# Kaz-K/medical-image-editing

Measured on AMD Instinct MI355X. Metric: images/sec (train step, 256x256 2D slices), higher is better.
Workload: dtype f32

## Files before the change

medical-image-editing_amd/csrc/conv_wino64.hip:

```cpp
#include "common.h"
#include "conv_common.h"
#include "mfma_util.h"
#include "wino_common.h"

extern int g_wino_mode;

namespace {

struct W64Args {
    const float* x;
    const float* u;
    const float* bias;
    float* y;
    int N, H, W, Cin, Cout;
    int tilesY, tilesX, nsp;
    int ntn, nch;
    int kt;
    int relu;
    unsigned nbx, nbu, nby;
    float* stats;
    const float* mask;
    const float* mr;
    int in_relu;
    float* y2;
    int split, pool0;
    int c1;
    unsigned nby2;
    unsigned img_px, rowb_px, rpx, ppx;
    int n_sh, n_m;
};

constexpr int W6_KPH = wino::KPH;
template <int RW, int MBW, int NW = 8> struct W64Geo {
    static_assert(MBW == 1 || (MBW == 2 && RW == 32), "two M blocks per wave: 32-wide regions only");
    static_assert(NW == 8 || (NW == 4 && RW == 32), "four-wave workgroups: 32-wide regions only");
    static constexpr int NMB = NW / 2;
    static constexpr int NBW = 4 / MBW;
    static constexpr int NCO = 16 * NBW;
    static constexpr int TR = RW == 32 ? 2 * MBW * NMB : 16;
    static constexpr int HR = TR + 2, HWV = RW + 2;
    static constexpr int HWS = RW == 32 ? 34 : 24;
    static constexpr int HBUF = HR * HWS * W6_KPH;
    static constexpr int UBUF = 16 * NCO * 8;
    static constexpr int EXF = 2048 * NW;
    static_assert(EXF >= UBUF, "U buffer 1 lives in the exchange area");
    static constexpr size_t LDS_FLOATS = 2 * HBUF + UBUF + EXF + 2 * NMB * NCO * 2;
};
constexpr int W6_LS = 4;
constexpr int W6_ULS = 2;
constexpr int W6_CP = 48;

template <int RW, int MBW, int EPI, int NW = 8>
__global__ void __launch_bounds__(64 * NW, 8 / NW) k_conv_wino64(W64Args a) {
    constexpr bool MASK = EPI >= 1 && EPI <= 3;
    using G = W64Geo<RW, MBW, NW>;
    constexpr int NT = 64 * NW, NMB = G::NMB, NBW = G::NBW, NCO = G::NCO;
    constexpr int HWS = G::HWS, HWV = G::HWV, HBUF = G::HBUF, UBUF = G::UBUF;
    using Halo = wino::HaloStager<NT, G::HR, HWV, HWS, wino::PitchedPix>;
    constexpr int LH = Halo::LH;
    constexpr int LU = 512 * NBW / NT;
    constexpr int HP0 = 1 + LU * W6_ULS;
    static_assert(HP0 + (LH - 1) * W6_LS < W6_CP && W6_CP + LH <= 64, "prefetch slots fit the item");

    extern __shared__ __attribute__((aligned(16))) float smem[];
    float* Hs = smem;
    float* Us = smem + 2 * HBUF;
    float* Ex = Us + UBUF;
    float* Rs = Ex + G::EXF;

    const int tid = threadIdx.x, lane = tid & 63;
    const int wv = __builtin_amdgcn_readfirstlane(tid >> 6);
    const int mb = wv & (NMB - 1), h = wv / NMB;
    const int H = a.H, W = a.W, Cin = a.Cin, Cout = a.Cout;
    const __amdgpu_buffer_rsrc_t rsx = make_rsrc(a.x, a.nbx), rsu = make_rsrc(a.u, a.nbu), rsy = make_rsrc(a.y, a.nby);
    const __amdgpu_buffer_rsrc_t rsm = make_rsrc((EPI == 1 || EPI == 3) ? a.mask : a.y, a.nby);
    const __amdgpu_buffer_rsrc_t rsr = make_rsrc(EPI == 3 ? a.mr : a.y, EPI == 3 ? (unsigned)((size_t)a.N * a.Cout * 8) : a.nby);
    const __amdgpu_buffer_rsrc_t rsy2 = make_rsrc(EPI == 4 ? a.y2 : a.y, EPI == 4 ? a.nby2 : a.nby);

    const int nch = a.nch;
    const wino::RegionRun run = wino::region_run(a.ntn, a.kt, a.nsp);
    const int co_base = run.tile_n * NCO;
    const int my_tiles = run.my_tiles;
    if (my_tiles <= 0) return;

    const int c4 = tid & 1;
    const wino::PitchedPix pixel = {a.img_px, a.rowb_px, a.rpx, a.ppx, a.n_sh, a.n_m};
    Halo hs;
    hs.init(tid, pixel);
    auto region_offsets = [&](int n, int tx, int ty) { hs.region_offsets(n, ty * G::TR - 1, tx * RW - 1, H, W, Cin); };
    const int u_n = (tid >> 1) & (NCO - 1);
    const int u_swz = (u_n >> 3) & 1;
    const int u_c4 = c4 ^ u_swz;
    const unsigned u_voff = (((unsigned)(tid >> 1) / NCO * Cout + co_base + u_n) * 8u + u_c4 * 4) * 4u;
    const unsigned u_jstride = (unsigned)(NT / 2 / NCO) * Cout * 32u;
    const unsigned u_cstride = 16u * Cout * 32u;
    const int u_wave = wv * 256;

    auto issue_h = [&](int j, int chunk) { hs.issue_h(rsx, j, chunk); };
    auto commit_h = [&](int j, float* Hb) { hs.commit_h(j, Hb); };
    auto issue_u = [&](int j, int chunk, float* Ub) {
        wino::buf_ld4_lds(rsu, Ub + u_wave + j * (NT * 4), u_voff, chunk * u_cstride + j * u_jstride);
    };

    int cn, ctx, cty, ch = 0;
    region_start(run.sp0, a.tilesY, a.tilesX, cn, ctx, cty);
    auto advance = [&](int& n, int& tx, int& ty, int& c) {
        const int adv = c + 1 == nch ? 1 : 0;
        c = adv ? 0 : c + 1;
        region_step(adv, a.tilesY, a.tilesX, n, tx, ty);
    };
    int n1 = cn, tx1 = ctx, ty1 = cty, ch1 = 0;
    advance(n1, tx1, ty1, ch1);
    int n2 = n1, tx2 = tx1, ty2 = ty1, ch2 = ch1;
    advance(n2, tx2, ty2, ch2);
    auto shift = [&]() {
        cn = n1; ctx = tx1; cty = ty1; ch = ch1;
        n1 = n2; tx1 = tx2; ty1 = ty2; ch1 = ch2;
        advance(n2, tx2, ty2, ch2);
    };

    const int m = lane & 15, q = lane >> 4;
    const int rA = h ? 3 : 0, rB = h ? 2 : 1, rC = h ? 1 : 2;
    const int prow = RW == 32 ? 2 * MBW * mb : 2 * (2 * mb + (m >> 3)), pcol = RW == 32 ? 2 * m : 2 * (m & 7);
    constexpr int MBW_STEP = 2 * HWS * W6_KPH;
    const int a_A = opaque(((prow + rA) * HWS + pcol) * W6_KPH + 2 * q);
    const int a_B = opaque(((prow + rB) * HWS + pcol) * W6_KPH + 2 * q);
    const int a_C = opaque(((prow + rC) * HWS + pcol) * W6_KPH + 2 * q);
    const int b_swz = ((q >> 1) ^ (m >> 3)) * 4 + (q & 1) * 2;
    const int b_0 = opaque(((h ? 3 : 0) * 4 * NCO + m) * 8 + b_swz);
    const int b_1 = opaque(((h ? 2 : 1) * 4 * NCO + m) * 8 + b_swz);
    const float sg = opaque_f(h ? -1.f : 1.f), mone = opaque_f(-1.f);

    f32x4 acc[8][MBW][NBW];
    f32x2 bf[2][NBW];
    f32x2 dcol[2][3];
    float e[2][2][4];
    float v[2][MBW][2][8];

    auto read_col = [&](const float* Hb, int w, int c) {
        const float* Hc = Hb + w * MBW_STEP + c * W6_KPH;
        dcol[c & 1][0] = *(const f32x2*)&Hc[a_A];
        dcol[c & 1][1] = *(const f32x2*)&Hc[a_B];
        dcol[c & 1][2] = *(const f32x2*)&Hc[a_C];
    };
    auto xform_op = [&](int par, int w, int o) {
        if (o < 16) {
            const int c = o >> 2, k = o & 3, t = k >> 1;
            const float dA = dcol[c & 1][0][t], dB = dcol[c & 1][1][t], dC = dcol[c & 1][2][t];
            if ((k & 1) == 0) e[t][0][c] = __builtin_fmaf(mone, dC, dA);
            else e[t][1][c] = __builtin_fmaf(sg, dC, dB);
        } else {
            const int k = o - 16, lr = k >> 3, t = (k >> 2) & 1, cc = k & 3;
            const float e0 = e[t][lr][0], e1 = e[t][lr][1], e2 = e[t][lr][2], e3 = e[t][lr][3];
            v[par][w][t][lr * 4 + cc] = wino::bt_row_plain(cc, e0, e1, e2, e3);
        }
    };
    auto xform_slot = [&](const float* Hn, int par, int p) {
        constexpr int NOPS = 32 * MBW, P0 = MBW == 1 ? 32 : 4;
        auto op = [&](int g) { xform_op(par, g >> 5, g & 31); };
        auto rd = [&](int g) {
            if ((g & 31) < 16 && ((g & 31) & 3) == 0) read_col(Hn, g >> 5, (g & 31) >> 2);
        };
        if (p + 3 - P0 >= 0 && p + 3 - P0 < NOPS) rd(p + 3 - P0);
        if (p - P0 >= 0 && p - P0 < NOPS && p < 64) {
            const int g = p - P0;
            if (P0 + NOPS <= 64 || g < NOPS - 2 * (P0 + NOPS - 64)) op(g);
            else { const int d = g - (NOPS - 2 * (P0 + NOPS - 64)); op(NOPS - 2 * (P0 + NOPS - 64) + 2 * d); op(NOPS - 2 * (P0 + NOPS - 64) + 2 * d + 1); }
        }
    };

    region_offsets(cn, ctx, cty);
#pragma unroll
    for (int j = 0; j < LH; ++j) issue_h(j, 0);
#pragma unroll
    for (int j = 0; j < LU; ++j) issue_u(j, 0, Us);
#pragma unroll
    for (int j = 0; j < LH; ++j) commit_h(j, Hs);
    region_offsets(n1, tx1, ty1);
#pragma unroll
    for (int j = 0; j < LH; ++j) issue_h(j, ch1);
#pragma unroll
    for (int j = 0; j < LH; ++j) commit_h(j, Hs + HBUF);
    wino::dma_wait();
    __syncthreads();
#pragma unroll
    for (int w = 0; w < MBW; ++w)
#pragma unroll
        for (int o = 0; o < 32; ++o) {
            if (o < 16 && (o & 3) == 0) read_col(Hs, w, o >> 2);
            xform_op(0, w, o);
        }
    __syncthreads();
    region_offsets(n2, tx2, ty2);

    float bvv[NBW / 2];
#pragma unroll
    for (int i = 0; i < NBW / 2; ++i) bvv[i] = a.bias ? a.bias[co_base + (h * (NBW / 2) + i) * 16 + m] : 0.f;
    const float lo = a.relu ? 0.f : -__builtin_inff();
    const bool plain = a.bias == nullptr && !a.relu;
    int spar = 0;

    auto body = [&](auto PAR, auto FIRST) {
        constexpr int par = decltype(PAR)::value;
        constexpr bool first = decltype(FIRST)::value;
        const float* Uc = Us + par * UBUF;
        const float* Hn = Hs + (par ^ 1) * HBUF;
        float* Hw = Hs + par * HBUF;
        float* Uw = Us + (par ^ 1) * UBUF;
        auto ldb = [&](int l, int nb) {
            bf[l & 1][nb] = *(const f32x2*)&Uc[(l < 4 ? b_0 : b_1) + ((l & 3) * NCO + nb * 16) * 8];
        };
        static_assert(par == 0 || (par ^ 1) == 0, "a region's last item (odd) loads U into buffer 0: buffer 1 is the epilogue's exchange area");
        auto slot = [&](int p) {
            if (p >= 1 && p < HP0 && (p - 1) % W6_ULS == 0) issue_u((p - 1) / W6_ULS, ch1, Uw);
            if (p >= HP0 && p < HP0 + LH * W6_LS && (p - HP0) % W6_LS == 0) issue_h((p - HP0) / W6_LS, ch2);
            if (p >= W6_CP && p < W6_CP + LH) commit_h(p - W6_CP, Hw);
            xform_slot(Hn, par ^ 1, p);
        };
#pragma unroll
        for (int nb = 0; nb < NBW; ++nb) { ldb(0, nb); __builtin_amdgcn_sched_barrier(0); }
        const f32x4 zero4 = {0.f, 0.f, 0.f, 0.f};
        if (first) {
#pragma unroll
            for (int p = 0; p < 8; ++p) slot(p);
#pragma unroll
            for (int w = 0; w < MBW; ++w)
#pragma unroll
                for (int nb = 0; nb < NBW; ++nb) acc[7][w][nb] = zero4;
        } else {
#pragma unroll
            for (int j = 0; j < 8; ++j) {
                const int w = j / (2 * NBW), k = (j / NBW) & 1, nb = j % NBW;
                acc[7][w][nb] = MFMA16(v[par ^ 1][w][k][7], k == 0 ? bf[1][nb].x : bf[1][nb].y, acc[7][w][nb]);
                slot(j);
                __builtin_amdgcn_sched_barrier(0);
            }
        }
#pragma unroll
        for (int l = 0; l < 7; ++l) {
#pragma unroll
            for (int j = 0; j < 8; ++j) {
                const int w = j / (2 * NBW), k = (j / NBW) & 1, nb = j % NBW;
                if (j < NBW) ldb(l + 1, nb);
                acc[l][w][nb] = MFMA16(v[par][w][k][l], k == 0 ? bf[l & 1][nb].x : bf[l & 1][nb].y, (first && k == 0) ? zero4 : acc[l][w][nb]);
                slot(8 + l * 8 + j);
                __builtin_amdgcn_sched_barrier(0);
            }
        }
    };
    auto flush = [&]() {
#pragma unroll
        for (int j = 0; j < 8; ++j) {
            const int w = j / (2 * NBW), k = (j / NBW) & 1, nb = j % NBW;
            acc[7][w][nb] = MFMA16(v[1][w][k][7], k == 0 ? bf[1][nb].x : bf[1][nb].y, acc[7][w][nb]);
            __builtin_amdgcn_sched_barrier(0);
        }
    };

    auto partial = [&](auto HH, int w, int nb, int r, float* yv) {
        constexpr int hh = decltype(HH)::value;
        float p0[4], p1[4];
#pragma unroll
        for (int j = 0; j < 4; ++j) {
            const float l0 = acc[j][w][nb][r], l1 = acc[4 + j][w][nb][r];
            if (hh == 0) { p0[j] = l0 + l1; p1[j] = l1; }
            else { p0[j] = l1; p1[j] = l0 - l1; }
        }
        yv[0] = (p0[0] + p0[1]) + p0[2];
        yv[1] = (p0[1] - p0[2]) - p0[3];
        yv[2] = (p1[0] + p1[1]) + p1[2];
        yv[3] = (p1[1] - p1[2]) - p1[3];
    };
    auto epi_send = [&](auto HH) {
        constexpr int hh = decltype(HH)::value;
        float* Xo = Ex + (((mb * 2 + (hh ^ 1)) * 8) * 64 + lane) * 4;
#pragma unroll
        for (int w = 0; w < MBW; ++w)
#pragma unroll
            for (int i = 0; i < NBW / 2; ++i)
#pragma unroll
                for (int r = 0; r < 4; ++r) {
                    float yv[4];
                    partial(HH, w, (hh ^ 1) * (NBW / 2) + i, r, yv);
                    float4 o;
                    o.x = yv[0]; o.y = yv[1]; o.z = yv[2]; o.w = yv[3];
                    *(float4*)&Xo[((w * (NBW / 2) + i) * 4 + r) * 256] = o;
                }
    };
    auto epi_finish = [&](auto HH) {
        constexpr int hh = decltype(HH)::value;
        const float* Xi = Ex + (((mb * 2 + hh) * 8) * 64 + lane) * 4;
        float st1[NBW / 2], st2[NBW / 2];
#pragma unroll
        for (int w = 0; w < MBW; ++w) {
            const int yrow0 = cty * G::TR + (RW == 32 ? 2 * (MBW * mb + w) : 2 * (2 * mb + (q >> 1)));
            const int xcol0 = ctx * RW + (RW == 32 ? 8 * q : 8 * (q & 1));
#pragma unroll
            for (int i = 0; i < NBW / 2; ++i) {
                float yv[16];
                const int co0 = co_base + (hh * (NBW / 2) + i) * 16;
                const unsigned co = (unsigned)(co0 + m);
                const bool part0 = EPI == 4 && co0 < a.split;
                const bool pooled = part0 && a.pool0;
                const unsigned cs = EPI != 4 ? (unsigned)Cout : (unsigned)(part0 ? a.split : a.c1);
                const unsigned cc = EPI != 4 ? co : (part0 ? co : co - (unsigned)a.split);
                int voffs[2];
#pragma unroll
                for (int aa = 0; aa < 2; ++aa) {
                    const int yy = yrow0 + aa;
                    const unsigned base = (pixel.base(cn) + (unsigned)yy * a.rpx + (unsigned)xcol0 * a.ppx) * cs + cc;
                    voffs[aa] = (int)sel_u32(yy < H, base * 4u, 0xFFFFFFFFu);
                }
                float mk[16];
                if (MASK) {
#pragma unroll
                    for (int aa = 0; aa < 2; ++aa)
#pragma unroll
                        for (int r = 0; r < 4; ++r)
#pragma unroll
                            for (int b = 0; b < 2; ++b)
                                mk[r * 4 + aa * 2 + b] = __uint_as_float(__builtin_amdgcn_raw_buffer_load_b32(rsm, voffs[aa], (2 * r + b) * (int)a.ppx * Cout * 4, 0));
                }
#pragma unroll
                for (int r = 0; r < 4; ++r) {
                    float own[4];
                    partial(HH, w, hh * (NBW / 2) + i, r, own);
                    const float4 o = *(const float4*)&Xi[((w * (NBW / 2) + i) * 4 + r) * 256];
                    if (plain) {
                        yv[r * 4 + 0] = own[0] + o.x; yv[r * 4 + 1] = own[1] + o.y;
                        yv[r * 4 + 2] = own[2] + o.z; yv[r * 4 + 3] = own[3] + o.w;
                    } else {
                        yv[r * 4 + 0] = fmaxf((own[0] + o.x) + bvv[i], lo);
                        yv[r * 4 + 1] = fmaxf((own[1] + o.y) + bvv[i], lo);
                        yv[r * 4 + 2] = fmaxf((own[2] + o.z) + bvv[i], lo);
                        yv[r * 4 + 3] = fmaxf((own[3] + o.w) + bvv[i], lo);
                    }
                }
                if (EPI == 1) {
#pragma unroll
                    for (int k = 0; k < 16; ++k) yv[k] = mk[k] > 0.f ? yv[k] : 0.f;
                } else if (EPI == 2) {
#pragma unroll
                    for (int k = 0; k < 16; ++k) yv[k] = mk[k] + yv[k];
                } else if (EPI == 3) {
                    const unsigned mo = ((unsigned)(cn >> a.n_sh) * (unsigned)Cout + co) * 8u;
                    const float mean = __uint_as_float(__builtin_amdgcn_raw_buffer_load_b32(rsr, (int)mo, 0, 0));
                    const float rstd = __uint_as_float(__builtin_amdgcn_raw_buffer_load_b32(rsr, (int)mo, 4, 0));
                    float s1 = 0.f, s2 = 0.f;
#pragma unroll
                    for (int k = 0; k < 16; ++k) {
                        const float xh = (mk[k] - mean) * rstd;
                        const float gm = (a.in_relu && !(xh > 0.f)) ? 0.f : yv[k];
                        s1 += gm;
                        s2 = __builtin_fmaf(gm, xh, s2);
                    }
                    s1 += __shfl_xor(s1, 16, 64); s2 += __shfl_xor(s2, 16, 64);
                    s1 += __shfl_xor(s1, 32, 64); s2 += __shfl_xor(s2, 32, 64);
                    if (w == 0) { st1[i] = s1; st2[i] = s2; }
                    else { st1[i] += s1; st2[i] += s2; }
                }
                if (EPI == 4 && !part0 && co0 - a.split >= a.c1) {
                } else if (EPI == 4 && pooled) {
                    const unsigned base = (((unsigned)cn * (unsigned)(H >> 1) + (unsigned)(yrow0 >> 1)) * (unsigned)(W >> 1) + (unsigned)(xcol0 >> 1)) * cs + cc;
                    const int voff = (int)sel_u32(yrow0 < H, base * 4u, 0xFFFFFFFFu);
#pragma unroll
                    for (int r = 0; r < 4; ++r) {
                        const float t = (yv[r * 4 + 0] + yv[r * 4 + 1]) + (yv[r * 4 + 2] + yv[r * 4 + 3]);
                        __builtin_amdgcn_raw_buffer_store_b32(__float_as_uint(t), rsy, voff, r * (int)cs * 4, 0);
                    }
                } else {
#pragma unroll
                    for (int aa = 0; aa < 2; ++aa) {
                        const int voff = voffs[aa];
#pragma unroll
                        for (int r = 0; r < 4; ++r)
#pragma unroll
                            for (int b = 0; b < 2; ++b)
                                __builtin_amdgcn_raw_buffer_store_b32(__float_as_uint(yv[r * 4 + aa * 2 + b]), (EPI == 4 && !part0) ? rsy2 : rsy, voff,
                                                                      (2 * r + b) * (int)(a.ppx * cs) * 4, 0);
                    }
                }
                if (EPI != 3 && a.stats) {
                    float t1, t2;
                    lane_stats<16>(yv, t1, t2);
                    stat_merge_eq(t1, t2, __shfl_xor(t1, 16, 64), __shfl_xor(t2, 16, 64), 1.f / 32.f);
                    stat_merge_eq(t1, t2, __shfl_xor(t1, 32, 64), __shfl_xor(t2, 32, 64), 1.f / 64.f);
                    if (w == 0) { st1[i] = t1; st2[i] = t2; }
                    else stat_merge_eq(st1[i], st2[i], t1, t2, 1.f / 128.f);
                }
            }
        }
        if (a.stats && lane < 16) {
#pragma unroll
            for (int i = 0; i < NBW / 2; ++i) {
                float* R = Rs + spar * (NMB * NCO * 2) + (mb * NCO + (hh * (NBW / 2) + i) * 16 + lane) * 2;
                R[0] = st1[i];
                R[1] = st2[i];
            }
        }
    };
    auto fold_stats = [&]() {
        if (!a.stats) return;
        if (tid < NCO) {
            const float* R = Rs + spar * (NMB * NCO * 2) + tid * 2;
            float s1 = R[0], s2 = R[1];
            constexpr float PW = 64.f * MBW;
            if (EPI == 3) {
#pragma unroll
                for (int r = 1; r < NMB; ++r) { s1 += R[r * NCO * 2]; s2 += R[r * NCO * 2 + 1]; }
            } else {
#pragma unroll
                for (int r = 1; r < NMB; ++r) stat_merge(s1, s2, PW * r, R[r * NCO * 2], R[r * NCO * 2 + 1], PW);
            }
            const int t = (cn * a.tilesX + ctx) * a.tilesY + cty;
            float* o = a.stats + ((size_t)t * Cout + co_base + tid) * 2;
            o[0] = s1;
            o[1] = s2;
        }
        spar ^= 1;
    };

    using wino::P0;
    using wino::P1;
    auto item_end = [&]() {
        wino::dma_wait();
        __syncthreads();
    };
    for (int reg = 0; reg < my_tiles; ++reg) {
        body(P0{}, std::true_type{});
        item_end();
        shift();
        body(P1{}, std::false_type{});
        item_end();
        for (int c = 2; c < nch; c += 2) {
            shift();
            if (ch2 == 0) region_offsets(n2, tx2, ty2);
            body(P0{}, std::false_type{});
            item_end();
            shift();
            body(P1{}, std::false_type{});
            item_end();
        }
        flush();
        if (h == 0) epi_send(P0{}); else epi_send(P1{});
        __syncthreads();
        if (h == 0) epi_finish(P0{}); else epi_finish(P1{});
        __syncthreads();
        fold_stats();
        shift();
        if (ch2 == 0) region_offsets(n2, tx2, ty2);
    }
}

}

static int wino64_shape(int Cin, int Cout, int W) {
    if (Cin % 16 != 0) return 0;
    if (Cout % 64 == 0) return 1;
    return (Cout % 32 == 0 && W % 32 == 0) ? 2 : 0;
}
static int wino64_waves(int shape) { return shape == 2 ? 4 : 8; }
bool conv_wino64_ok(int Cin, int Cout, int W) { return wino64_shape(Cin, Cout, W) != 0; }
int conv_wino64_stat_tiles(int Cin, int Cout, int H, int W) {
    const int shape = wino64_shape(Cin, Cout, W);
    const int rw = W % 32 == 0 ? 32 : 16, tr = rw == 32 ? shape * wino64_waves(shape) : 16;
    return tr > 0 && H % tr == 0 ? (H / tr) * (W / rw) : 0;
}

template <int RW, int MBW, int EPI, int NW = 8>
static int launch_wino64(W64Args& a, hipStream_t st) {
    using G = W64Geo<RW, MBW, NW>;
    constexpr size_t lds = G::LDS_FLOATS * sizeof(float);
    static_assert(lds * (8 / NW) <= 160 * 1024, "buffers do not fit the 160 KB LDS");
    if (int rc = lds_opt_in<k_conv_wino64<RW, MBW, EPI, NW>>((int)lds, "conv_wino64")) return rc;
    a.tilesY = ceil_div(a.H, G::TR); a.tilesX = a.W / RW; a.nsp = a.N * a.tilesY * a.tilesX;
    a.ntn = a.Cout / G::NCO;
    a.kt = conv_region_runs(a.nsp, a.ntn, 8 / NW);
    k_conv_wino64<RW, MBW, EPI, NW><<<ceil_div(a.nsp, a.kt) * a.ntn, 64 * NW, lds, st>>>(a);
    VQW_LAUNCH_CHECK("conv_wino64");
    return VQW_OK;
}

bool conv_wino64_dil2_ok(int Cin, int Cout, int H, int W) {
    return H % 2 == 0 && W % 64 == 0 && wino64_shape(Cin, Cout, W / 2) != 0;
}
int conv_wino64_fwd(const float* x, const float* u, const float* bias, float* y, int N, int H, int W, int Cin, int Cout, int relu,
                    hipStream_t st, float* stats, const float* mask, int accumulate, const float* in_mr, int in_relu, int dil) {
    W64Args a;
    const long P = (long)N * H * W;
    a.img_px = (unsigned)(H * W); a.rowb_px = 0; a.rpx = (unsigned)W; a.ppx = 1; a.n_sh = 0; a.n_m = 0;
    if (dil == 2) {
        a.rowb_px = (unsigned)W; a.rpx = 2u * (unsigned)W; a.ppx = 2; a.n_sh = 2; a.n_m = 1;
        N *= 4; H /= 2; W /= 2;
    }
    a.y2 = nullptr; a.split = 0; a.pool0 = 0; a.c1 = 0; a.nby2 = 0;
    a.x = x; a.u = u; a.bias = bias; a.y = y; a.mask = mask; a.mr = in_mr; a.in_relu = in_relu;
    a.N = N; a.H = H; a.W = W; a.Cin = Cin; a.Cout = Cout;
    a.nch = Cin / 8;
    a.relu = relu;
    a.stats = stats;
    a.nbx = (unsigned)(P * Cin * 4);
    a.nbu = (unsigned)(16L * Cout * Cin * 4);
    a.nby = (unsigned)(P * Cout * 4);
    const int shape = wino64_shape(Cin, Cout, W);
    if (in_mr) {
        if (shape == 2) return launch_wino64<32, 2, 3, 4>(a, st);
        if (W % 32 == 0) return launch_wino64<32, 1, 3>(a, st);
        return launch_wino64<16, 1, 3>(a, st);
    }
    if (mask) {
        if (shape == 2) return launch_wino64<32, 2, 1, 4>(a, st);
        if (W % 32 == 0) return launch_wino64<32, 1, 1>(a, st);
        return launch_wino64<16, 1, 1>(a, st);
    }
    if (accumulate) {
        if (shape == 2) return launch_wino64<32, 2, 2, 4>(a, st);
        if (W % 32 == 0) return launch_wino64<32, 1, 2>(a, st);
        return launch_wino64<16, 1, 2>(a, st);
    }
    if (shape == 2) return launch_wino64<32, 2, 0, 4>(a, st);
    if (W % 32 == 0) return launch_wino64<32, 1, 0>(a, st);
    return launch_wino64<16, 1, 0>(a, st);
}

bool conv_wino64_split_ok(int Cin, int Cout, int split, int pool0, int N, int H, int W, int c1) {
    if (c1 < 0 || c1 % 16 != 0 || split + c1 > Cout) return false;
    if (!conv_wino64_ok(Cin, Cout, W) || g_wino_mode != 0 || split <= 0 || split >= Cout || split % 16 != 0) return false;
    if (pool0 && (H % 2 != 0)) return false;
    return (long)N * H * W * (Cin > Cout ? Cin : Cout) * 4 <= 0xFFFFFFE0L;
}
int conv_wino64_fwd_split(const float* x, const float* u, const float* bias, float* y0, float* y1, int N, int H, int W, int Cin, int Cout,
                          int split, int pool0, int relu, hipStream_t st, int c1) {
    if (c1 <= 0) c1 = Cout - split;
    W64Args a;
    a.img_px = (unsigned)(H * W); a.rowb_px = 0; a.rpx = (unsigned)W; a.ppx = 1; a.n_sh = 0; a.n_m = 0;
    a.x = x; a.u = u; a.bias = bias; a.y = y0; a.y2 = y1; a.mask = nullptr; a.mr = nullptr; a.in_relu = 0;
    a.split = split; a.pool0 = pool0; a.c1 = c1;
    a.N = N; a.H = H; a.W = W; a.Cin = Cin; a.Cout = Cout;
    a.nch = Cin / 8;
    a.relu = relu;
    a.stats = nullptr;
    const long P = (long)N * H * W;
    a.nbx = (unsigned)(P * Cin * 4);
    a.nbu = (unsigned)(16L * Cout * Cin * 4);
    a.nby = (unsigned)((pool0 ? P / 4 : P) * split * 4);
    a.nby2 = (unsigned)(P * c1 * 4);
    const int shape = wino64_shape(Cin, Cout, W);
    if (shape == 2) return launch_wino64<32, 2, 4, 4>(a, st);
    if (W % 32 == 0) return launch_wino64<32, 1, 4>(a, st);
    return launch_wino64<16, 1, 4>(a, st);
}

namespace {

struct W64WgArgs {
    const float* x;
    const float* dy;
    float* part;
    float* bias_part;
    int N, H, W, Cin, Cout;
    int tilesY, tilesX, nsp;
    int n_ci_b, nblk, kt;
    unsigned nbx, nbd;
    const float* x1;
    int C0, up0;
    unsigned nbx1;
    unsigned img_px, rowb_px, rpx, ppx;
    int n_sh, n_m;
};

constexpr int W6_WLS = 2;
constexpr int WG_XP = 40;
template <int RW, int MB> struct WgGeo {
    static_assert((MB == 4 && (RW == 32 || RW == 16)) || (MB == 2 && RW == 32), "the 16-wide region needs the dense rows of the 64-cout form");
    static constexpr int DP = 16 * MB + 8;
    static constexpr int TRP = RW == 32 ? 4 : 8;
    static constexpr int XW = RW + 2, XR = TRP + 2, XPIX = XR * XW;
    static constexpr int DBUF = 128 * DP, XBUF = XPIX * WG_XP;
    static constexpr size_t LDS_BYTES = (size_t)2 * (DBUF + XBUF) * sizeof(float);
    static_assert(LDS_BYTES <= 160 * 1024 && LDS_BYTES >= 64 * 1024, "tiles fit the LDS; the fold needs 64 KB");
};

template <int RW, int MB>
__global__ void __launch_bounds__(512, 1) k_conv_wino_wgrad_blk(W64WgArgs a) {
    using G = WgGeo<RW, MB>;
    constexpr int NT = 512, DP = G::DP, DBUF = G::DBUF, XBUF = G::XBUF, XW = G::XW;
    constexpr int XF = G::XPIX * 8;
    constexpr int LX = (XF + NT - 1) / NT;
    constexpr int QD = 4 * MB;
    constexpr int DPX = NT / QD, LD = MB;
    constexpr int NP = 8 * MB;
    constexpr bool PITCH = MB == 2;
    extern __shared__ __attribute__((aligned(16))) float smem[];

    const int tid = threadIdx.x, lane = tid & 63;
    const int wv = __builtin_amdgcn_readfirstlane(tid >> 6);
    const int r = wv & 3, kh = wv >> 2;
    const int H = a.H, W = a.W, Cin = a.Cin, Cout = a.Cout;
    const int lb = xcd_remap(blockIdx.x, gridDim.x);
    const int blk = lb % a.nblk, sblk = lb / a.nblk;
    const int co_base = (blk / a.n_ci_b) * (16 * MB), ci_base = (blk % a.n_ci_b) * 32;
    const int sp0 = sblk * a.kt;
    const int my_tiles = min(a.kt, a.nsp - sp0);
    const bool do_bias = a.bias_part != nullptr && ci_base == 0;
    const unsigned rpx = PITCH ? a.rpx : (unsigned)W, ppx = PITCH ? a.ppx : 1u;

    const int d_px = tid / QD;
    const unsigned d_fix = (((unsigned)(d_px / RW) * rpx + (unsigned)(d_px % RW) * ppx) * Cout + co_base + (tid % QD) * 4) * 4u;
    const unsigned d_jstride = (unsigned)(DPX / RW) * rpx * Cout * 4u;
    const int d_lds = d_px * DP + (tid % QD) * 4;
    const bool x_s1 = ci_base >= a.C0;
    const bool x_up = !x_s1 && a.up0;
    const float* x_ptr = x_s1 ? a.x1 : a.x;
    const int x_cs = x_s1 ? Cin - a.C0 : a.C0, x_cb = x_s1 ? ci_base - a.C0 : ci_base;
    const int x_w = x_up ? W >> 1 : W, x_h = x_up ? H >> 1 : H;
    const long x_nb = x_s1 ? (long)a.nbx1 : (long)a.nbx;
    const unsigned x_rpx = x_up ? (unsigned)x_w : rpx, x_ppx = x_up ? 1u : ppx;
    unsigned x_fix[LX];
    int x_lds[LX];
    unsigned x_bits = 0;
#pragma unroll
    for (int j = 0; j < LX; ++j) {
        int f = tid + j * NT;
        if (f >= XF) f -= XF;
        const int hp = f >> 3, hy = hp / XW, hx = hp - hy * XW;
        x_fix[j] = (((unsigned)(x_up ? (hy + 1) >> 1 : hy) * x_rpx + (unsigned)(x_up ? (hx + 1) >> 1 : hx) * x_ppx) * x_cs + x_cb + (tid & 7) * 4) * 4u;
        x_lds[j] = 2 * DBUF + hp * WG_XP + (tid & 7) * 4;
        x_bits |= (unsigned)((hy == 0 ? 1 : 0) | (hy == G::XR - 1 ? 2 : 0) | (hx == 0 ? 4 : 0) | (hx == XW - 1 ? 8 : 0)) << (4 * j);
    }
    float4 rd[LD], rx[LX];
    float4 bsum;
    bsum.x = bsum.y = bsum.z = bsum.w = 0.f;
    __amdgpu_buffer_rsrc_t rsd, rsx;
    unsigned x_edges = 0;
    auto region_setup = [&](int n, int tx, int ty) {
        const int y0 = ty * G::TRP, x0 = tx * RW;
        long dpix;
        if constexpr (PITCH) {
            const long nbase = (long)(n >> a.n_sh) * a.img_px + (long)((n >> 1) & a.n_m) * a.rowb_px + (n & a.n_m);
            dpix = nbase + (long)y0 * a.rpx + (long)x0 * a.ppx;
        } else {
            dpix = ((long)n * H + y0) * W + x0;
        }
        const long doff = dpix * Cout * 4;
        rsd = __builtin_amdgcn_make_buffer_rsrc((void*)((const char*)a.dy + doff), 0, (int)(unsigned)((long)a.nbd - doff), 0x00020000);
        const long xpix = x_up ? ((long)n * x_h + (y0 >> 1) - 1) * x_w + (x0 >> 1) - 1
                               : PITCH ? dpix - (long)a.rpx - (long)a.ppx : dpix - W - 1;
        const long xoff = xpix * x_cs * 4;
        const long xleft = x_nb - xoff;
        rsx = __builtin_amdgcn_make_buffer_rsrc((void*)((const char*)x_ptr + xoff), 0, (int)(unsigned)(xleft > 0xFFFFFFF0L ? 0xFFFFFFF0L : xleft), 0x00020000);
        x_edges = ((y0 == 0 ? 1u : 0u) | (y0 + G::TRP == H ? 2u : 0u) | (x0 == 0 ? 4u : 0u) | (x0 + RW == W ? 8u : 0u)) * 0x1111u;
    };
    auto issue_d = [&](int j) { rd[j] = buf_ld4(rsd, d_fix, j * d_jstride); };
    auto issue_x = [&](int j) {
        const unsigned vo = (x_bits & x_edges & (0xFu << (4 * j))) ? 0xFFFFFFFFu : x_fix[j];
        rx[j] = buf_ld4(rsx, vo, 0);
    };
    float once_v = 1.f;
    auto commit_d = [&](int j, int buf) {
        *(float4*)&smem[d_lds + buf * DBUF + j * DPX * DP] = rd[j];
        if (do_bias) {
            bsum.x = __builtin_fmaf(once_v, rd[j].x, bsum.x); bsum.y = __builtin_fmaf(once_v, rd[j].y, bsum.y);
            bsum.z = __builtin_fmaf(once_v, rd[j].z, bsum.z); bsum.w = __builtin_fmaf(once_v, rd[j].w, bsum.w);
        }
    };
    auto commit_x = [&](int j, int buf) { *(float4*)&smem[x_lds[j] + buf * XBUF] = rx[j]; };

    const int idx = lane & 15, k = lane >> 4;
    const int aF = r == 3 ? 1 : 0, aS = r == 0 ? 0 : 1;
    const int trow0 = RW == 32 ? kh : 2 * kh;
    const int a_F = opaque(((2 * trow0 + aF) * RW + 2 * k) * DP + idx);
    const int a_S = opaque(((2 * trow0 + aS) * RW + 2 * k) * DP + idx);
    const int iA = r == 0 ? 0 : r == 2 ? 2 : 1, iB = r == 0 ? 2 : r == 1 ? 2 : r == 2 ? 1 : 3;
    const int x_A = opaque(2 * DBUF + ((2 * trow0 + iA) * XW + 2 * k) * WG_XP + idx);
    const int x_B = opaque(2 * DBUF + ((2 * trow0 + iB) * XW + 2 * k) * WG_XP + idx);
    const float sA = opaque_f((r == 1) ? 1.f : (r == 2) ? -1.f : 0.f), sB = opaque_f((r == 1) ? 1.f : -1.f);
    auto s_px_d = [](int s) { return RW == 32 ? 8 * s : 2 * (s >> 1) * 16 + 8 * (s & 1); };
    auto s_px_x = [](int s) { return RW == 32 ? 8 * s : 2 * (s >> 1) * XW + 8 * (s & 1); };

    f32x4 acc[4][MB][2];
#pragma unroll
    for (int c = 0; c < 4; ++c)
#pragma unroll
        for (int mb = 0; mb < MB; ++mb)
#pragma unroll
            for (int nb = 0; nb < 2; ++nb)
#pragma unroll
                for (int q = 0; q < 4; ++q) acc[c][mb][nb][q] = 0.f;
    float dm[2][MB][4];
    float vv[2][2][4];
    float ra[2][4], rb[2][8];

    auto rd_grp = [&](int nbuf, int s, int g, int i) {
        if (g < MB) {
            const int o = nbuf * DBUF + s_px_d(s) * DP + g * 16 + (i & 1) * DP;
            ra[g & 1][i] = i < 2 ? smem[a_F + o] : smem[a_S + o];
        } else {
            const int o = nbuf * XBUF + s_px_x(s) * WG_XP + (g - MB) * 16 + (i & 3) * WG_XP;
            rb[g & 1][i] = i < 4 ? smem[x_A + o] : smem[x_B + o];
        }
    };
    auto op_grp = [&](int set, int g, int i) {
        if (g < MB) {
            float* d = dm[set][g];
            const float* q = ra[g & 1];
            if (i == 0) d[0] = __builtin_fmaf(sA, q[2], q[0]);
            if (i == 1) d[3] = __builtin_fmaf(sA, q[3], q[1]);
            if (i == 2) d[1] = d[0] + d[3];
            if (i == 3) d[2] = d[0] - d[3];
        } else {
            float* o = vv[set][g - MB];
            float* q = rb[g & 1];
            if (i < 4) q[i] = __builtin_fmaf(sB, q[4 + i], q[i]);
            if (i == 4) o[0] = q[0] - q[2];
            if (i == 5) o[1] = q[1] + q[2];
            if (i == 6) o[2] = q[2] - q[1];
            if (i == 7) o[3] = q[1] - q[3];
        }
    };
    auto build_slot = [&](int nbuf, int s, int set, int p) {
        if constexpr (MB == 4) {
            if (p < 4) rd_grp(nbuf, s, 0, p);
            else if (p < 16) { op_grp(set, (p - 4) >> 2, (p - 4) & 3); rd_grp(nbuf, s, ((p - 4) >> 2) + 1, (p - 4) & 3); }
            else if (p < 20) { op_grp(set, 3, p - 16); rd_grp(nbuf, s, 4, 2 * (p - 16)); rd_grp(nbuf, s, 4, 2 * (p - 16) + 1); }
            else if (p < 28) { op_grp(set, 4, p - 20); rd_grp(nbuf, s, 5, p - 20); }
            else { op_grp(set, 5, 2 * (p - 28)); op_grp(set, 5, 2 * (p - 28) + 1); }
        } else {
            auto rd2 = [&](int g, int i0) { rd_grp(nbuf, s, g, i0); rd_grp(nbuf, s, g, i0 + 1); };
            auto op2 = [&](int g, int i0) { op_grp(set, g, i0); op_grp(set, g, i0 + 1); };
            if (p == 0) rd2(0, 0);
            else if (p == 1) rd2(0, 2);
            else if (p == 2) rd2(1, 0);
            else if (p == 3) { op2(0, 0); rd2(1, 2); }
            else if (p == 4) { op2(0, 2); rd2(2, 0); }
            else if (p == 5) { op2(1, 0); rd2(2, 2); }
            else if (p == 6) { op2(1, 2); rd2(2, 4); }
            else if (p == 7) rd2(2, 6);
            else if (p < 12) { op2(2, 2 * (p - 8)); rd2(3, 2 * (p - 8)); }
            else op2(3, 2 * (p - 12));
        }
    };

    int cn, ctx, cty;
    region_start(sp0, a.tilesY, a.tilesX, cn, ctx, cty);
    if (my_tiles > 0) {
        region_setup(cn, ctx, cty);
#pragma unroll
        for (int j = 0; j < LD; ++j) issue_d(j);
#pragma unroll
        for (int j = 0; j < LX; ++j) issue_x(j);
#pragma unroll
        for (int j = 0; j < LD; ++j) commit_d(j, 0);
#pragma unroll
        for (int j = 0; j < LX; ++j) commit_x(j, 0);
        __syncthreads();
#pragma unroll
        for (int p = 0; p < NP; ++p) build_slot(0, 0, 0, p);
    }
    int ln = cn, ltx = ctx, lty = cty, lcount = 0;
    auto load_advance = [&]() {
        if (lcount + 1 < my_tiles) { region_next(a.tilesY, a.tilesX, ln, ltx, lty); ++lcount; once_v = 1.f; } else once_v = 0.f;
        region_setup(ln, ltx, lty);
    };
    if (my_tiles > 0) {
        load_advance();
#pragma unroll
        for (int j = 0; j < LD; ++j) issue_d(j);
    }

    auto phase = [&](auto SET, auto SNEXT, auto NBUF, auto DBUFW, auto LOADS) {
        constexpr int set = decltype(SET)::value, sn = decltype(SNEXT)::value, nbuf = decltype(NBUF)::value;
        constexpr int wbuf = decltype(DBUFW)::value, loads = decltype(LOADS)::value;
#pragma unroll
        for (int c = 0; c < 4; ++c)
#pragma unroll
            for (int mb = 0; mb < MB; ++mb)
#pragma unroll
                for (int nb = 0; nb < 2; ++nb) {
                    const int p = c * 2 * MB + mb * 2 + nb;
                    acc[c][mb][nb] = MFMA16(dm[set][mb][c], vv[set][nb][c], acc[c][mb][nb]);
                    build_slot(nbuf, sn, set ^ 1, p);
                    if (loads == 0 && p >= 8 && p < 8 + LD) commit_d(p - 8, wbuf);
                    if (loads == 1 && p >= 2 && p < 2 + W6_WLS * LX && (p - 2) % W6_WLS == 0) issue_x((p - 2) / W6_WLS);
                    if (loads == 2 && p >= 8 && p < 8 + LX) commit_x(p - 8, wbuf);
                    if (loads == 3 && p >= 2 && p < 2 + W6_WLS * LD && (p - 2) % W6_WLS == 0) issue_d((p - 2) / W6_WLS);
                    __builtin_amdgcn_sched_barrier(0);
                }
    };
    using I0 = std::integral_constant<int, 0>;
    using I1 = std::integral_constant<int, 1>;
    using I2 = std::integral_constant<int, 2>;
    using I3 = std::integral_constant<int, 3>;
    auto region = [&](auto BUF) {
        constexpr int b = decltype(BUF)::value;
        using B = std::integral_constant<int, b>;
        using NB = std::integral_constant<int, b ^ 1>;
        phase(I0{}, I1{}, B{}, NB{}, I0{});
        phase(I1{}, I2{}, B{}, NB{}, I1{});
        phase(I0{}, I3{}, B{}, NB{}, I2{});
        __syncthreads();
        load_advance();
        phase(I1{}, I0{}, NB{}, B{}, I3{});
    };
    for (int g = 0; g < my_tiles; g += 2) {
        region(I0{});
        if (g + 1 < my_tiles) region(I1{});
    }

    __syncthreads();
    float* red = smem;
    if (do_bias) {
        *(float4*)&red[tid * 4] = bsum;
        __syncthreads();
        if (tid < 16 * MB) {
            const int cq = tid >> 2, comp = tid & 3;
            float sum = 0.f;
            for (int i = 0; i < DPX; ++i) sum += red[(i * QD + cq) * 4 + comp];
            a.bias_part[(size_t)sblk * Cout + co_base + tid] = sum;
        }
        __syncthreads();
    }
    int fold_w = ((kh * 4 + r) * 4 * 16 + 4 * (lane >> 4)) * 32 + idx, fold_r = tid;
    asm volatile("" : "+v"(fold_w), "+v"(fold_r));
#pragma unroll
    for (int mb = 0; mb < MB; ++mb) {
#pragma unroll
        for (int c = 0; c < 4; ++c)
#pragma unroll
            for (int nb = 0; nb < 2; ++nb)
#pragma unroll
                for (int q = 0; q < 4; ++q)
                    red[fold_w + c * 512 + q * 32 + nb * 16] = acc[c][mb][nb][q];
        __syncthreads();
        {
            const int e = fold_r;
            float tcol[3][4];
#pragma unroll
            for (int c = 0; c < 4; ++c) {
                float u[4];
#pragma unroll
                for (int rr = 0; rr < 4; ++rr) {
                    const float t = red[((0 * 4 + rr) * 4 + c) * 512 + e] + red[((1 * 4 + rr) * 4 + c) * 512 + e];
                    u[rr] = ((rr == 3) != (c == 3)) ? -t : t;
                }
                tcol[0][c] = u[0] + 0.5f * (u[1] + u[2]);
                tcol[1][c] = 0.5f * (u[1] - u[2]);
                tcol[2][c] = u[3] + 0.5f * (u[1] + u[2]);
            }
            const int co = co_base + mb * 16 + (tid >> 5), ci = ci_base + (tid & 31);
            float* o = a.part + (size_t)sblk * Cout * 9 * Cin + ((size_t)co * 9) * Cin + ci;
#pragma unroll
            for (int ky = 0; ky < 3; ++ky) {
                const float t0 = tcol[ky][0], t1 = tcol[ky][1], t2 = tcol[ky][2], t3 = tcol[ky][3];
                o[(ky * 3 + 0) * Cin] = t0 + 0.5f * (t1 + t2);
                o[(ky * 3 + 1) * Cin] = 0.5f * (t1 - t2);
                o[(ky * 3 + 2) * Cin] = t3 + 0.5f * (t1 + t2);
            }
        }
        __syncthreads();
    }
}

}

static int wgrad_blk_mb(int C0, int C1, int up0, int Cout, int H, int W) {
    if (C1 == 0 ? (up0 || C0 % 32 != 0)
                : (C0 % 32 != 0 || C1 % 32 != 0 || (up0 && (H % 2 != 0 || W % 2 != 0)))) return 0;
    if (Cout % 64 == 0) return (W % 16 == 0 && H % (W % 32 == 0 ? 4 : 8) == 0) ? 4 : 0;
    return (Cout % 32 == 0 && W % 32 == 0 && H % 4 == 0) ? 2 : 0;
}
bool conv_wino_blk_wgrad_ok(int C0, int C1, int up0, int Cout, int H, int W) { return wgrad_blk_mb(C0, C1, up0, Cout, H, W) != 0; }
bool conv_wino_blk_wgrad_dil2_ok(int C0, int Cout, int H, int W) {
    return H % 2 == 0 && W % 2 == 0 && wgrad_blk_mb(C0, 0, 0, Cout, H / 2, W / 2) == 2;
}
int conv_wino_blk_wgrad_blocks(int Cin, int Cout, int N, int H, int W, int max_slabs, int* kt_out) {
    const int rw = W % 32 == 0 ? 32 : 16;
    return conv_slab_split(N * (H / (128 / rw)) * (W / rw), (Cout / (Cout % 64 == 0 ? 64 : 32)) * (Cin / 32), max_slabs, kt_out);
}
template <int RW, int MB>
static int launch_wgrad_blk(const W64WgArgs& a, int nsb, hipStream_t st) {
    if (int rc = lds_opt_in<k_conv_wino_wgrad_blk<RW, MB>>(160 * 1024, "conv_wino_blk_wgrad")) return rc;
    k_conv_wino_wgrad_blk<RW, MB><<<a.nblk * nsb, 512, WgGeo<RW, MB>::LDS_BYTES, st>>>(a);
    VQW_LAUNCH_CHECK("conv_wino_blk_wgrad");
    return VQW_OK;
}
int conv_wino_blk_wgrad(const ConvIn& in, const float* dy, float* ws, float* bpart, int N, int H, int W, int Cin, int Cout, int nsb, int kt,
                        hipStream_t st, int dil) {
    const long P = (long)N * H * W;
    W64WgArgs a;
    a.dy = dy; a.part = ws; a.bias_part = bpart;
    a.Cin = Cin; a.Cout = Cout;
    a.x = in.src0; a.x1 = in.C1 ? in.src1 : in.src0; a.C0 = in.C0; a.up0 = in.C1 ? in.up0 : 0;
    a.nbx = (unsigned)((a.up0 ? P / 4 : P) * in.C0 * 4);
    a.nbx1 = (unsigned)(P * in.C1 * 4);
    a.nbd = (unsigned)(P * Cout * 4);
    a.img_px = (unsigned)(H * W); a.rowb_px = 0; a.rpx = (unsigned)W; a.ppx = 1; a.n_sh = 0; a.n_m = 0;
    if (dil == 2) {
        a.rowb_px = (unsigned)W; a.rpx = 2u * (unsigned)W; a.ppx = 2; a.n_sh = 2; a.n_m = 1;
        N *= 4; H /= 2; W /= 2;
    }
    a.N = N; a.H = H; a.W = W;
    const int rw = W % 32 == 0 ? 32 : 16, mb = Cout % 64 == 0 ? 4 : 2;
    a.tilesY = H / (128 / rw); a.tilesX = W / rw; a.nsp = N * a.tilesY * a.tilesX;
    a.n_ci_b = Cin / 32; a.nblk = (Cout / (16 * mb)) * a.n_ci_b; a.kt = kt;
    if (mb == 2) return launch_wgrad_blk<32, 2>(a, nsb, st);
    return rw == 32 ? launch_wgrad_blk<32, 4>(a, nsb, st) : launch_wgrad_blk<16, 4>(a, nsb, st);
}
```

medical-image-editing_amd/csrc/wino_common.h:

```cpp
#pragma once
#include "mfma_util.h"
#include <type_traits>

namespace wino {

using P0 = std::integral_constant<int, 0>;
using P1 = std::integral_constant<int, 1>;

struct RegionRun {
    int tile_n, sp0, my_tiles;
};
__device__ __forceinline__ RegionRun region_run(int ntn, int kt, int nsp) {
    const int lb = xcd_remap(blockIdx.x, gridDim.x);
    RegionRun r;
    r.tile_n = lb % ntn;
    r.sp0 = (lb / ntn) * kt;
    r.my_tiles = min(kt, nsp - r.sp0);
    return r;
}

template <class Args>
struct ItemCursor {
    const Args& a;
    int cn, ctx, cty, ch;
    int n1, tx1, ty1, ch1;
    int n2, tx2, ty2, ch2;
    __device__ __forceinline__ void advance(int& n, int& tx, int& ty, int& c) const {
        const int adv = c + 1 == a.nch ? 1 : 0;
        c = adv ? 0 : c + 1;
        region_step(adv, a.tilesY, a.tilesX, n, tx, ty);
    }
    __device__ __forceinline__ ItemCursor(const Args& a_, int sp0) : a(a_) {
        region_start(sp0, a.tilesY, a.tilesX, cn, ctx, cty);
        ch = 0;
        n1 = cn; tx1 = ctx; ty1 = cty; ch1 = 0;
        advance(n1, tx1, ty1, ch1);
        n2 = n1; tx2 = tx1; ty2 = ty1; ch2 = ch1;
        advance(n2, tx2, ty2, ch2);
    }
    __device__ __forceinline__ void shift() {
        cn = n1; ctx = tx1; cty = ty1; ch = ch1;
        n1 = n2; tx1 = tx2; ty1 = ty2; ch1 = ch2;
        advance(n2, tx2, ty2, ch2);
    }
};

template <class Cursor, class Body, class Offsets, class Epilogue>
__device__ __forceinline__ void region_loop(int my_tiles, int nch, Cursor& it, Body&& body, Offsets&& offsets, Epilogue&& epilogue) {
    for (int reg = 0; reg < my_tiles; ++reg) {
        body(P0{}, std::true_type{});
        __syncthreads();
        it.shift();
        body(P1{}, std::false_type{});
        __syncthreads();
        for (int c = 2; c < nch; c += 2) {
            it.shift();
            if (it.ch2 == 0) offsets(it.n2, it.tx2, it.ty2);
            body(P0{}, std::false_type{});
            __syncthreads();
            it.shift();
            body(P1{}, std::false_type{});
            __syncthreads();
        }
        epilogue();
        it.shift();
        if (it.ch2 == 0) offsets(it.n2, it.tx2, it.ty2);
    }
}

struct DensePix {
    unsigned H, W;
    __device__ __forceinline__ unsigned operator()(int n, int yy, int xx) const { return ((unsigned)n * H + (unsigned)yy) * W + (unsigned)xx; }
};
struct PitchedPix {
    unsigned img_px, rowb_px, rpx, ppx;
    int n_sh, n_m;
    __device__ __forceinline__ unsigned base(int n) const {
        return (unsigned)(n >> n_sh) * img_px + (unsigned)((n >> 1) & n_m) * rowb_px + (unsigned)(n & n_m);
    }
    __device__ __forceinline__ unsigned operator()(int n, int yy, int xx) const { return base(n) + (unsigned)yy * rpx + (unsigned)xx * ppx; }
};

constexpr int KPH = 10;

template <int NT, int HR, int HWV, int HWS, class Pix>
struct HaloStager {
    static constexpr int HF = HR * HWV * 2;
    static constexpr int LH = (HF + NT - 1) / NT;
    static_assert(HF > (LH - 1) * NT && HF >= NT, "every halo slot but the last is full");
    Pix pix;
    int tid, c4;
    int h_lds[LH];
    unsigned h_voff[LH];
    float4 rh[LH];
    __device__ __forceinline__ void halo_pixel(int j, int& hy, int& hx) const {
        int f = tid + j * NT;
        if (f >= HF) f -= HF;
        const int hp = f >> 1;
        hy = hp / HWV;
        hx = hp - hy * HWV;
    }
    __device__ __forceinline__ void init(int tid_, const Pix& pix_) {
        tid = tid_; c4 = tid_ & 1; pix = pix_;
#pragma unroll
        for (int j = 0; j < LH; ++j) {
            int hy, hx;
            halo_pixel(j, hy, hx);
            h_lds[j] = (hy * HWS + hx) * KPH + c4 * 4;
        }
    }
    __device__ __forceinline__ void region_offsets(int n, int y0, int x0, int H, int W, int C) {
#pragma unroll
        for (int j = 0; j < LH; ++j) {
            int hy, hx;
            halo_pixel(j, hy, hx);
            const int yy = y0 + hy, xx = x0 + hx;
            const bool ok = ((unsigned)yy < (unsigned)H) & ((unsigned)xx < (unsigned)W);
            h_voff[j] = sel_u32(ok, pix(n, yy, xx) * (unsigned)C * 4u + (unsigned)c4 * 16u, 0xFFFFFFFFu);
        }
    }
    __device__ __forceinline__ void issue_h(__amdgpu_buffer_rsrc_t rs, int j, int chunk) { rh[j] = buf_ld4(rs, h_voff[j], chunk * 32); }
    __device__ __forceinline__ void commit_h(int j, float* Hb) {
        float* p = Hb + h_lds[j];
        f32x2 lo, hi;
        lo.x = rh[j].x; lo.y = rh[j].y; hi.x = rh[j].z; hi.y = rh[j].w;
        *(f32x2*)p = lo;
        *(f32x2*)(p + 2) = hi;
    }
};

__device__ __forceinline__ void buf_ld4_lds(__amdgpu_buffer_rsrc_t r, float* lds_wave, unsigned byte_off, unsigned soff) {
    __builtin_amdgcn_raw_ptr_buffer_load_lds(r, (__attribute__((address_space(3))) void*)lds_wave, 16, (int)byte_off, (int)soff, 0, 0);
}
__device__ __forceinline__ void dma_wait() { __builtin_amdgcn_s_waitcnt(0x0F70); }

__device__ __forceinline__ float bt_row(int r, float d0, float d1, float d2, float d3, float pone, float mone) {
    return r == 0 ? __builtin_fmaf(mone, d2, d0) : r == 1 ? __builtin_fmaf(pone, d2, d1) : r == 2 ? __builtin_fmaf(mone, d1, d2) : __builtin_fmaf(mone, d3, d1);
}
__device__ __forceinline__ float bt_row_plain(int r, float d0, float d1, float d2, float d3) {
    return r == 0 ? d0 - d2 : r == 1 ? d1 + d2 : r == 2 ? d2 - d1 : d1 - d3;
}

__device__ __forceinline__ void weight_transform(const double g[3][3], double u[4][4]) {
    double t[4][3];
    for (int kx = 0; kx < 3; ++kx) {
        t[0][kx] = g[0][kx];
        t[1][kx] = 0.5 * (g[0][kx] + g[1][kx] + g[2][kx]);
        t[2][kx] = 0.5 * (g[0][kx] - g[1][kx] + g[2][kx]);
        t[3][kx] = g[2][kx];
    }
    for (int i = 0; i < 4; ++i) {
        u[i][0] = t[i][0];
        u[i][1] = 0.5 * (t[i][0] + t[i][1] + t[i][2]);
        u[i][2] = 0.5 * (t[i][0] - t[i][1] + t[i][2]);
        u[i][3] = t[i][2];
    }
}

}
```

Measured before the change: 361.9.

## Load Winograd halo tiles directly into LDS via buffer-load DMA

For the 32-wide, eight-wave Winograd conv configuration, halo input tiles are now loaded straight into LDS with buffer_load...lds instead of going through registers and a later LDS store. The halo layout changes to pixel pairs padded to 5 dwords-per-lane units, and column addressing is adjusted to match. This removes VGPR staging and the ds_write commit slots, which frees registers and instruction issue in the pipelined loop. In exchange it adds padded LDS slots, clamped duplicate pieces and a new bank pattern for reads, and it relies on the existing DMA wait to cover the halo loads.

Result: no change. 362.8, median of 6 (+0.2%).

```diff
diff --git a/medical-image-editing_amd/csrc/conv_wino64.hip b/medical-image-editing_amd/csrc/conv_wino64.hip
--- a/medical-image-editing_amd/csrc/conv_wino64.hip
+++ b/medical-image-editing_amd/csrc/conv_wino64.hip
@@ -40,7 +40,10 @@
     static constexpr int TR = RW == 32 ? 2 * MBW * NMB : 16;
     static constexpr int HR = TR + 2, HWV = RW + 2;
     static constexpr int HWS = RW == 32 ? 34 : 24;
-    static constexpr int HBUF = HR * HWS * W6_KPH;
+    static constexpr bool HDMA = RW == 32 && NW == 8;
+    using Halo = std::conditional_t<HDMA, wino::HaloDma<NW, HR, HWV, HWS, wino::PitchedPix>,
+                                    wino::HaloStager<64 * NW, HR, HWV, HWS, wino::PitchedPix>>;
+    static constexpr int HBUF = HDMA ? wino::HaloDma<NW, HR, HWV, HWS, wino::PitchedPix>::BUF : HR * HWS * W6_KPH;
     static constexpr int UBUF = 16 * NCO * 8;
     static constexpr int EXF = 2048 * NW;
     static_assert(EXF >= UBUF, "U buffer 1 lives in the exchange area");
@@ -55,12 +58,13 @@
     constexpr bool MASK = EPI >= 1 && EPI <= 3;
     using G = W64Geo<RW, MBW, NW>;
     constexpr int NT = 64 * NW, NMB = G::NMB, NBW = G::NBW, NCO = G::NCO;
-    constexpr int HWS = G::HWS, HWV = G::HWV, HBUF = G::HBUF, UBUF = G::UBUF;
-    using Halo = wino::HaloStager<NT, G::HR, HWV, HWS, wino::PitchedPix>;
+    constexpr int HWS = G::HWS, HBUF = G::HBUF, UBUF = G::UBUF;
+    using Halo = typename G::Halo;
+    constexpr bool HD = G::HDMA;
     constexpr int LH = Halo::LH;
     constexpr int LU = 512 * NBW / NT;
     constexpr int HP0 = 1 + LU * W6_ULS;
-    static_assert(HP0 + (LH - 1) * W6_LS < W6_CP && W6_CP + LH <= 64, "prefetch slots fit the item");
+    static_assert(HP0 + (LH - 1) * W6_LS < (HD ? 64 : W6_CP) && W6_CP + LH <= 64, "prefetch slots fit the item");
 
     extern __shared__ __attribute__((aligned(16))) float smem[];
     float* Hs = smem;
@@ -86,7 +90,7 @@
     const int c4 = tid & 1;
     const wino::PitchedPix pixel = {a.img_px, a.rowb_px, a.rpx, a.ppx, a.n_sh, a.n_m};
     Halo hs;
-    hs.init(tid, pixel);
+    if constexpr (HD) hs.init(tid, wv, pixel); else hs.init(tid, pixel);
     auto region_offsets = [&](int n, int tx, int ty) { hs.region_offsets(n, ty * G::TR - 1, tx * RW - 1, H, W, Cin); };
     const int u_n = (tid >> 1) & (NCO - 1);
     const int u_swz = (u_n >> 3) & 1;
@@ -96,8 +100,12 @@
     const unsigned u_cstride = 16u * Cout * 32u;
     const int u_wave = wv * 256;
 
-    auto issue_h = [&](int j, int chunk) { hs.issue_h(rsx, j, chunk); };
-    auto commit_h = [&](int j, float* Hb) { hs.commit_h(j, Hb); };
+    auto issue_h = [&](int j, int chunk, float* Hb) {
+        if constexpr (HD) hs.issue_h(rsx, j, chunk, Hb); else hs.issue_h(rsx, j, chunk);
+    };
+    auto commit_h = [&](int j, float* Hb) {
+        if constexpr (!HD) hs.commit_h(j, Hb);
+    };
     auto issue_u = [&](int j, int chunk, float* Ub) {
         wino::buf_ld4_lds(rsu, Ub + u_wave + j * (NT * 4), u_voff, chunk * u_cstride + j * u_jstride);
     };
@@ -138,7 +146,7 @@
     float v[2][MBW][2][8];
 
     auto read_col = [&](const float* Hb, int w, int c) {
-        const float* Hc = Hb + w * MBW_STEP + c * W6_KPH;
+        const float* Hc = Hb + w * MBW_STEP + (HD ? wino::halo_dma_col(c) : c * W6_KPH);
         dcol[c & 1][0] = *(const f32x2*)&Hc[a_A];
         dcol[c & 1][1] = *(const f32x2*)&Hc[a_B];
         dcol[c & 1][2] = *(const f32x2*)&Hc[a_C];
@@ -171,14 +179,14 @@
 
     region_offsets(cn, ctx, cty);
 #pragma unroll
-    for (int j = 0; j < LH; ++j) issue_h(j, 0);
+    for (int j = 0; j < LH; ++j) issue_h(j, 0, Hs);
 #pragma unroll
     for (int j = 0; j < LU; ++j) issue_u(j, 0, Us);
 #pragma unroll
     for (int j = 0; j < LH; ++j) commit_h(j, Hs);
     region_offsets(n1, tx1, ty1);
 #pragma unroll
-    for (int j = 0; j < LH; ++j) issue_h(j, ch1);
+    for (int j = 0; j < LH; ++j) issue_h(j, ch1, Hs + HBUF);
 #pragma unroll
     for (int j = 0; j < LH; ++j) commit_h(j, Hs + HBUF);
     wino::dma_wait();
@@ -213,8 +221,8 @@
         static_assert(par == 0 || (par ^ 1) == 0, "a region's last item (odd) loads U into buffer 0: buffer 1 is the epilogue's exchange area");
         auto slot = [&](int p) {
             if (p >= 1 && p < HP0 && (p - 1) % W6_ULS == 0) issue_u((p - 1) / W6_ULS, ch1, Uw);
-            if (p >= HP0 && p < HP0 + LH * W6_LS && (p - HP0) % W6_LS == 0) issue_h((p - HP0) / W6_LS, ch2);
-            if (p >= W6_CP && p < W6_CP + LH) commit_h(p - W6_CP, Hw);
+            if (p >= HP0 && p < HP0 + LH * W6_LS && (p - HP0) % W6_LS == 0) issue_h((p - HP0) / W6_LS, ch2, Hw);
+            if (!HD && p >= W6_CP && p < W6_CP + LH) commit_h(p - W6_CP, Hw);
             xform_slot(Hn, par ^ 1, p);
         };
 #pragma unroll
diff --git a/medical-image-editing_amd/csrc/wino_common.h b/medical-image-editing_amd/csrc/wino_common.h
--- a/medical-image-editing_amd/csrc/wino_common.h
+++ b/medical-image-editing_amd/csrc/wino_common.h
@@ -134,6 +134,35 @@
 }
 __device__ __forceinline__ void dma_wait() { __builtin_amdgcn_s_waitcnt(0x0F70); }
 
+constexpr int halo_dma_col(int c) { return (c >> 1) * 2 * KPH + (c & 1) * 8; }
+template <int NW, int HR, int HWV, int HWS, class Pix>
+struct HaloDma {
+    static_assert(HWS % 2 == 0 && HWV <= HWS, "rows of whole pixel pairs");
+    static constexpr int RU = HWS / 2 * 5;
+    static constexpr int NP = (HR * RU + 63) / 64;
+    static constexpr int LH = (NP + NW - 1) / NW;
+    static constexpr int BUF = NP * 256;
+    Pix pix;
+    int lane, wv;
+    unsigned h_voff[LH];
+    __device__ __forceinline__ int piece(int j) const { return min(wv + j * NW, NP - 1); }
+    __device__ __forceinline__ void init(int tid, int wv_, const Pix& pix_) { lane = tid & 63; wv = wv_; pix = pix_; }
+    __device__ __forceinline__ void region_offsets(int n, int y0, int x0, int H, int W, int C) {
+#pragma unroll
+        for (int j = 0; j < LH; ++j) {
+            const int u = piece(j) * 64 + lane;
+            const int hy = u / RU, r = u - hy * RU, pr = r / 5, k = r - pr * 5;
+            const int hx = 2 * pr + (k >> 1);
+            const int yy = y0 + hy, xx = x0 + hx;
+            const bool ok = (k < 4) & (hx < HWV) & (hy < HR) & ((unsigned)yy < (unsigned)H) & ((unsigned)xx < (unsigned)W);
+            h_voff[j] = sel_u32(ok, pix(n, yy, xx) * (unsigned)C * 4u + (unsigned)(k & 1) * 16u, 0xFFFFFFFFu);
+        }
+    }
+    __device__ __forceinline__ void issue_h(__amdgpu_buffer_rsrc_t rs, int j, int chunk, float* Hb) const {
+        buf_ld4_lds(rs, Hb + piece(j) * 256, h_voff[j], chunk * 32);
+    }
+};
+
 __device__ __forceinline__ float bt_row(int r, float d0, float d1, float d2, float d3, float pone, float mone) {
     return r == 0 ? __builtin_fmaf(mone, d2, d0) : r == 1 ? __builtin_fmaf(pone, d2, d1) : r == 2 ? __builtin_fmaf(mone, d1, d2) : __builtin_fmaf(mone, d3, d1);
 }
```
